# EmbersArc/EiCOS

Hardware: NVIDIA B200
Metric: SOCP solves/sec (higher is better)
Workload: dtype f64

## Files before the change

### eicos_b200/csrc/engine.cu

```cuda
#include "engine.hpp"
#include "backend.hpp"
#include "tile_program.hpp"

#include <algorithm>
#include <cstdint>
#ifdef EICOS_EMU
#include <thread>
#endif

namespace eicos
{

#ifndef EICOS_EMU
#define EI_DEFINE_KERNEL(name, fn, minblocks) EI_DEFINE_KERNEL_(name, fn, EI_MAX_THREADS, minblocks, 0)
#define EI_DEFINE_KERNEL1(name, fn) EI_DEFINE_KERNEL_(name, fn, 32, 8, 0)
#define EI_DEFINE_KERNEL_(name, fn, maxthreads, minblocks, JOBS)                                           \
    __global__ void __launch_bounds__(maxthreads, minblocks) name(const __grid_constant__ KArgs a) \
    {                                                                                          \
        extern __shared__ double smem[];                                                       \
        Team tm;                                                                               \
        tm.pl = threadIdx.x & 31;                                                              \
        tm.lane = tm.pl * VEC;                                                                 \
        tm.wk = threadIdx.x >> 5;                                                              \
        tm.nwk = blockDim.x >> 5;                                                              \
// ... 210 lines not shown
        P.Gp = upload(S.G.p, owned_, st);
        P.Gi = upload(S.G.i, owned_, st);
        P.Ap = upload(S.A.p, owned_, st);
        P.Ai = upload(S.A.i, owned_, st);
        P.Grp = upload(S.Gr.p, owned_, st);
        P.Grv = upload(S.Gr.v, owned_, st);
        P.Arp = upload(S.Ar.p, owned_, st);
        P.Arv = upload(S.Ar.v, owned_, st);
        P.cone_z = upload(S.cone_z, owned_, st);
    }
    P.cone_dim = upload(S.q, owned_, st);
    P.cone_k = upload(S.cone_k, owned_, st);
    P.cone_q = upload(S.cone_q, owned_, st);
    P.zk = upload(S.zk, owned_, st);
    P.xeq = dxeq_ = upload(S.xeq, owned_, st);
    P.Aeq = dAeq_ = upload(S.Aeq, owned_, st);
    P.GeqE = dGeq_ = upload(expanded_geq(S), owned_, st);
    const auto prog = [&](const MachineCode &h, DevMachine &d, int **keep = nullptr) {
        int *o = upload(h.ops, owned_, st);
        d.ops = o;
        d.nchunks = h.nchunks;
        d.nld_chunks = h.nld_chunks;
        d.ring_groups = h.ring_groups;
        d.ring_row0 = m_row_slot0(h.nr) + h.nr * h.slot_budget;
        if (keep)
            *keep = o;
    };
    const auto variant = [&](const ivec &list, std::initializer_list<int> va, std::initializer_list<int> vb = {}) {
        ivec out(list.size());
        int off[16] = {0};
        int k = 1;
        for (int o : va)
            off[k++] = o;
        k = 9;
        for (int o : vb)
            off[k++] = o;
        for (size_t q = 0; q < list.size(); q++)
        {
            const int w = list[q];
            out[q] = w == M_LD_NONE ? 0 : (w & M_LD_ROW_MASK) + off[(((unsigned)w >> M_LD_SEL_SHIFT) & 7) + ((w & M_LD_JOB_B) ? 8 : 0)];
        }
        return upload(out, owned_, st);
    };
    P.sw_budget = H_.fw[0].slot_budget;
    P.fa_budget = H_.fa[0].slot_budget;
    const int rhs[2] = {L_.rhs1, L_.rhs2}, sol[2] = {L_.sol1, L_.sol2}, xw[2] = {L_.xw, L_.xw2};
    const int dxr[2] = {L_.dxr, L_.dxr2}, er[2] = {L_.e, L_.e2};
    for (int v = 0; v < M_VARIANTS; v++)
    {
        prog(H_.fw[v], P.fw[v]);
        prog(H_.bw[v], P.bw[v]);
        prog(H_.bwp[v], P.bwp[v]);
        prog(H_.mv[v], P.mv[v], &dmv_ops_[v]);
        prog(H_.fa[v], P.fa[v], &dfa_ops_[v]);
        for (int set = 0; set < 2; set++)
        {
            P.fw_ld[v][set][0] = variant(H_.fw[v].ld, {rhs[set], 0, xw[set]});
            P.fw_ld[v][set][1] = variant(H_.fw[v].ld, {er[set], 0, xw[set]});
            P.bw_ld[v][set][0] = variant(H_.bwp[v].ld, {sol[set], 0, xw[set], rhs[set]});
            P.bw_ld[v][set][1] = variant(H_.bw[v].ld, {dxr[set], sol[set], xw[set], er[set]});
            P.mv_ld[v][set] = variant(H_.mv[v].ld, {rhs[set], sol[set], L_.lpv, er[set]});
        }
        P.fa_ld[v] = variant(H_.fa[v].ld, {});
    }
    for (int k = 0; k < M_MV_PARTS; k++)
    {
        prog(H_.rs[k], P.rs[k], &drs_ops_[k]);
        prog(H_.mvw[k], P.mvw[k], &dmvw_ops_[k]);
        P.rs_ld[k] = variant(H_.rs[k].ld, {L_.chb, L_.w, L_.s, L_.r, L_.sc});
        for (int set = 0; set < 2; set++)
            P.mvw_ld[set][k] = variant(H_.mvw[k].ld, {rhs[set], sol[set], L_.lpv, er[set]});
    }
    P.pair_budget = H_.pair_budget;
    prog(H_.fw2, P.fw2);
    prog(H_.bw2, P.bw2);
    prog(H_.bwp2, P.bwp2);
    prog(H_.mv2, P.mv2, &dmv2_ops_);
    P.fw2_ld[0] = variant(H_.fw2.ld, {rhs[0], 0, xw[0]}, {rhs[1], 0, xw[1]});
    P.fw2_ld[1] = variant(H_.fw2.ld, {er[0], 0, xw[0]}, {er[1], 0, xw[1]});
    P.bw2_ld[0] = variant(H_.bwp2.ld, {sol[0], 0, xw[0], rhs[0]}, {sol[1], 0, xw[1], rhs[1]});
    P.bw2_ld[1] = variant(H_.bw2.ld, {dxr[0], sol[0], xw[0], er[0]}, {dxr[1], sol[1], xw[1], er[1]});
    P.mv2_ld = variant(H_.mv2.ld, {rhs[0], sol[0], L_.lpv, er[0]}, {rhs[1], sol[1], L_.lpv, er[1]});
    P.mv_rows = H_.mv_rows;
    ivec vk;
    for (int k = 0; k < S.l; k++)
        vk.push_back(0);
    for (int d : S.q)
    {
        for (int k = 0; k < d + 1; k++)
            vk.push_back(0);
        for (int k = 1; k < d; k++)
            vk.push_back(1);
        vk.push_back(2);
        for (int k = 0; k < d; k++)
            vk.push_back(1);
    }
    P.Vkind = upload(vk, owned_, st);
    be::sync(st);
}

void Engine::upload_values(const Symbolic &S)
{
    be::stream_t st = S_(stream_);
    be::set_device(device_);
    refresh_stream_values(S, L_, H_, pim_);
    const dvec ge = expanded_geq(S);
    be::h2d(dxeq_, S.xeq.data(), S.xeq.size() * sizeof(double), st);
    be::h2d(dAeq_, S.Aeq.data(), S.Aeq.size() * sizeof(double), st);
    be::h2d(dGeq_, ge.data(), ge.size() * sizeof(double), st);
    for (int v = 0; v < M_VARIANTS; v++)
    {
        be::h2d(dmv_ops_[v], H_.mv[v].ops.data(), H_.mv[v].ops.size() * sizeof(int), st);
        be::h2d(dfa_ops_[v], H_.fa[v].ops.data(), H_.fa[v].ops.size() * sizeof(int), st);
    }
    be::h2d(dmv2_ops_, H_.mv2.ops.data(), H_.mv2.ops.size() * sizeof(int), st);
    for (int k = 0; k < M_MV_PARTS; k++)
    {
        be::h2d(drs_ops_[k], H_.rs[k].ops.data(), H_.rs[k].ops.size() * sizeof(int), st);
        be::h2d(dmvw_ops_[k], H_.mvw[k].ops.data(), H_.mvw[k].ops.size() * sizeof(int), st);
    }
    be::sync(st);
}

Engine::Engine(const Symbolic &S, int device, long long capacity_instances, int workers, bool instance_matrices)
    : device_(device), workers_(std::max(1, std::min(workers, EI_MAX_THREADS / 32 > 0 ? EI_MAX_THREADS / 32 : 1))),
      pim_(instance_matrices), nnzG_(S.G.nnz()), nnzA_(S.A.nnz())
{
    be::set_device(device_);
    if (const char *v = std::getenv("EICOS_RING_VARIANT"))
        force_variant_ = std::atoi(v);
    if (const char *v = std::getenv("EICOS_PAIR_SOLVES"))
        force_pair_ = std::atoi(v);
    if (const char *v = std::getenv("EICOS_WIDE"))
        force_wide_ = std::atoi(v);
    stream_ = (void *)(intptr_t)be::make_stream();
    build_layout(S, false);
    upload_pattern(S);
    cap_tiles_ = std::max<long long>(1, (capacity_instances + TILE - 1) / TILE);
    ws_bytes_ = (size_t)cap_tiles_ * L_.rows_total * TILE * sizeof(double);
    ws_ = (double *)be::alloc(ws_bytes_);
    const size_t ib = (size_t)cap_tiles_ * L_.irows_total * TILE * sizeof(int);
    iws_ = (int *)be::alloc(ib);
    be::zero(ws_, ws_bytes_, S_(stream_));
    be::zero(iws_, ib, S_(stream_));
    base_vec_ = (double *)be::alloc((size_t)(S.n + S.m + S.p) * sizeof(double));
    if (pim_)
        base_mat_ = (double *)be::alloc((size_t)(nnzG_ + nnzA_ + 1) * sizeof(double));
    active_count_ = (unsigned int *)be::alloc(sizeof(unsigned int));
    ir_rounds_ = (unsigned long long *)be::alloc(8 * sizeof(unsigned long long));
    host_pinned_ = (unsigned int *)be::pinned(12 * sizeof(unsigned long long));
    const size_t slots = (size_t)cap_tiles_ * TILE;
    moves_dev_ = (int *)be::alloc(2 * slots * sizeof(int));
    status_host_ = (int *)be::pinned(slots * sizeof(int));
    moves_host_ = (int *)be::pinned(2 * slots * sizeof(int));
    for (int v = 0; v < M_VARIANTS; v++)
    {
        const int sw_v = std::max(std::max(H_.fw[v].slot_budget, H_.bw[v].slot_budget), std::max(H_.bwp[v].slot_budget, H_.mv[v].slot_budget));
        smem_prog_[v] = machine_smem_doubles(sw_v, variant_groups(v)) * sizeof(double);
        smem_factor_[v] = machine_smem_doubles(P_.fa_budget, variant_groups(v)) * sizeof(double);
    }
    smem_pair_ = machine_smem_doubles(P_.pair_budget, M_PAIR_GROUPS, 2) * sizeof(double);
    part_doubles_ = machine_smem_doubles(P_.sw_budget, M_PART_GROUPS);
    smem_resid_ = part_doubles_ * sizeof(double);
    smem_wide_ = ((size_t)M_MV_PARTS * KRED * TILE +
                  std::max((size_t)M_MV_PARTS * part_doubles_, std::max(smem_prog_[0], smem_prog_[M_VARIANTS - 1]) / sizeof(double))) *
                 sizeof(double);
    smem_common_ = workers_ > 1 ? (size_t)workers_ * KRED * TILE * sizeof(double) : 0;
#ifndef EICOS_EMU
    {
        if (smem_pair_ > 48 * 1024)
            EI_CUDA(cudaFuncSetAttribute(eicos_solve_kkt_pair, cudaFuncAttributeMaxDynamicSharedMemorySize, (int)smem_pair_));
        if (smem_wide_ > 48 * 1024)
        {
            EI_CUDA(cudaFuncSetAttribute(eicos_solve_kkt_wide, cudaFuncAttributeMaxDynamicSharedMemorySize, (int)smem_wide_));
            EI_CUDA(cudaFuncSetAttribute(eicos_residuals_wide, cudaFuncAttributeMaxDynamicSharedMemorySize, (int)smem_wide_));
        }
        if (smem_resid_ > 48 * 1024)
            EI_CUDA(cudaFuncSetAttribute(eicos_residuals, cudaFuncAttributeMaxDynamicSharedMemorySize, (int)smem_resid_));
        const size_t top_f = std::max(smem_factor_[0], smem_factor_[M_VARIANTS - 1]), top_p = std::max(smem_prog_[0], smem_prog_[M_VARIANTS - 1]);
        if (top_f > 48 * 1024)
            EI_CUDA(cudaFuncSetAttribute(eicos_ldl_factor, cudaFuncAttributeMaxDynamicSharedMemorySize, (int)top_f));
        if (top_p > 48 * 1024)
        {
            EI_CUDA(cudaFuncSetAttribute(eicos_solve_kkt, cudaFuncAttributeMaxDynamicSharedMemorySize, (int)top_p));
            EI_CUDA(cudaFuncSetAttribute(eicos_residuals, cudaFuncAttributeMaxDynamicSharedMemorySize, (int)top_p));
        }
        int dev_sms = 148;
        EI_CUDA(cudaDeviceGetAttribute(&dev_sms, cudaDevAttrMultiProcessorCount, device_));
        sms_ = dev_sms;
    }
    if (smem_common_ > 48 * 1024)
    {
        const void *ks[] = {(const void *)eicos_load_inputs, (const void *)eicos_equilibrate, (const void *)eicos_init,
                            (const void *)eicos_init_point,
                            (const void *)eicos_iter_head, (const void *)eicos_iter_mid, (const void *)eicos_iter_tail,
                            (const void *)eicos_store_outputs};
        for (const void *k : ks)
            EI_CUDA(cudaFuncSetAttribute(k, cudaFuncAttributeMaxDynamicSharedMemorySize, (int)smem_common_));
    }
#endif
    be::sync(S_(stream_));
}

Engine::~Engine()
{
    be::set_device(device_);
#ifndef EICOS_EMU
    for (void *e : events_)
        cudaEventDestroy((cudaEvent_t)e);
#endif
    for (void *p : owned_)
        be::dfree(p);
    be::dfree(ws_);
    be::dfree(iws_);
    be::dfree(base_vec_);
    be::dfree(base_mat_);
    be::dfree(active_count_);
// ... 444 lines not shown
```

### eicos_b200/csrc/engine.hpp

```cpp
#pragma once

#include "layout.hpp"
#include "streams.hpp"
#include "symbolic.hpp"

#include <cstddef>
#include <vector>

namespace eicos
{

struct SolveStats
{
    int chunks = 0, compactions = 0;
    int ipm_iterations = 0;
    long long launches = 0;
    unsigned long long ir_rounds = 0;
    unsigned long long kkt_phase_cycles[5] = {0, 0, 0, 0, 0};
    double ms_total = 0, ms_factor = 0, ms_solve = 0, ms_other = 0;
    long long factor_launch_tiles = 0, solve_launch_tiles = 0;
    int factor_launches = 0, solve_launches = 0;
    double ms_resid = 0, ms_vector = 0;
    long long resid_launch_tiles = 0, vector_launch_tiles = 0;
    int resid_launches = 0, vector_launches = 0;
// ... 9 lines not shown
        factor_launch_tiles += o.factor_launch_tiles, solve_launch_tiles += o.solve_launch_tiles;
        factor_launches += o.factor_launches, solve_launches += o.solve_launches;
        ms_resid += o.ms_resid, ms_vector += o.ms_vector;
        resid_launch_tiles += o.resid_launch_tiles, vector_launch_tiles += o.vector_launch_tiles;
        resid_launches += o.resid_launches, vector_launches += o.vector_launches;
        lane_rounds += o.lane_rounds;
        return *this;
    }
};

struct ProgramStats
{
    int sw_slots = 0, fa_slots = 0, fa_fast = 0;
    long long sw_far = 0, sw_direct = 0, fa_home = 0;
    int fw_loads = 0, bw_loads = 0, fa_loads = 0, mv_loads = 0;
};

class Engine
{
  public:
    Engine(const Symbolic &S, int device, long long capacity_instances, int workers, bool instance_matrices = false);
    ~Engine();
    Engine(const Engine &) = delete;
    Engine &operator=(const Engine &) = delete;

    void set_matrices(const double *d_G, const double *d_A, const double *base_G, const double *base_A);
    bool instance_matrices() const { return pim_; }

    void upload_values(const Symbolic &S);

    void solve(int batch, const double *d_c, const double *d_h, const double *d_b,
               const double *base_c, const double *base_h, const double *base_b,
               double *d_x, double *d_y, double *d_z, double *d_s,
               int *d_exit, int *d_iter, double *d_info, int *d_iinfo,
               bool keep_sticky, bool pre_equilibrated, bool timing, SolveStats *stats);

    void debug_factor_init(int batch, const double *d_c, const double *d_h, const double *d_b,
                           const double *base_c, const double *base_h, const double *base_b,
                           double *h_Lx, double *h_D, double *h_sol1, double *h_sol2, int *h_nit);

    void debug_line_search(int batch, const double *h_lambda, const double *h_ds, const double *h_dz, const double *h_scalars,
                           double *h_alpha);

    ProgramStats program_stats() const;
    void *stream() const { return stream_; }
    int device() const { return device_; }
    int workers() const { return workers_; }
    void set_compaction(bool on) { compaction_ = on; }
    void set_iter_max(int k) { iter_max_ = k; }
    long long capacity() const { return cap_tiles_ * (long long)tile_width(); }
    size_t workspace_bytes() const { return ws_bytes_; }
    const Layout &layout() const { return L_; }
    static int tile_width();

  private:
    void build_layout(const Symbolic &S, bool acc_rows);
    void upload_pattern(const Symbolic &S);

    int device_ = 0, workers_ = 4;
    bool pim_ = false;
    const double *mat_dG_ = nullptr, *mat_dA_ = nullptr;
    double *base_mat_ = nullptr;
    int nnzG_ = 0, nnzA_ = 0;
    long long cap_tiles_ = 0;
    size_t ws_bytes_ = 0;
    void *stream_ = nullptr;
    Layout L_{};
    DevPattern P_{};
    double *ws_ = nullptr;
    int *iws_ = nullptr;
    double *base_vec_ = nullptr;
    unsigned int *active_count_ = nullptr;
    unsigned long long *ir_rounds_ = nullptr;
    unsigned int *host_pinned_ = nullptr;
    int *moves_dev_ = nullptr, *status_host_ = nullptr, *moves_host_ = nullptr;
    bool compaction_ = true;
    size_t smem_factor_[M_VARIANTS] = {0, 0}, smem_common_ = 0, smem_prog_[M_VARIANTS] = {0, 0};
    size_t smem_pair_ = 0;
    size_t smem_resid_ = 0, smem_wide_ = 0, part_doubles_ = 0;
    int force_wide_ = -1;
    int iter_max_ = Settings::iter_max;
    bool wide_launch(int ctas) const;
    int sms_ = 148, force_variant_ = -1, force_pair_ = -1;
    bool deep_ring(int ctas) const;
    bool pair_solves(int tiles) const;
    std::vector<void *> owned_;
    double *dxeq_ = nullptr, *dAeq_ = nullptr, *dGeq_ = nullptr;
    int *dmv_ops_[M_VARIANTS] = {nullptr, nullptr}, *drs_ops_[M_MV_PARTS] = {nullptr, nullptr, nullptr, nullptr}, *dmvw_ops_[M_MV_PARTS] = {nullptr, nullptr, nullptr, nullptr}, *dfa_ops_[M_VARIANTS] = {nullptr, nullptr}, *dmv2_ops_ = nullptr;
    HostStreams H_;
    std::vector<int> Lp_;
    std::vector<void *> events_;
};

}
```

### eicos_b200/csrc/layout.hpp

```cpp
#pragma once

#include <cstddef>

namespace eicos
{

enum : int
{
    ST_ACTIVE = -1000,
    EXIT_OPTIMAL = 0,
    EXIT_PINF = 1,
    EXIT_DINF = 2,
    EXIT_MAXIT = -1,
    EXIT_NUMERICS = -2,
    EXIT_OUTCONE = -3,
    EXIT_FATAL = -7,
    EXIT_INACC = 10,
    EXIT_NOT_CONVERGED = -87
};

enum ScalarRow : int
{
    S_KAP, S_TAU, S_CX, S_BY, S_HZ,
    S_PCOST, S_DCOST, S_PRES, S_DRES, S_PINFRES, S_DINFRES, S_GAP, S_RELGAP,
    S_SIGMA, S_MU, S_STEP, S_STEP_AFF, S_KAPOVERT,
    S_WORK_END,
    S_BEST = S_WORK_END,
    S_BEST_END = S_BEST + S_WORK_END,
    S_RT = S_BEST_END, S_NX, S_NY, S_NZ, S_NS, S_HRESX, S_HRESY, S_HRESZ,
    S_RESX0, S_RESY0, S_RESZ0, S_PRES_PREV,
    S_DTAU_DENOM, S_DTAUAFF, S_DKAPAFF,
    S_RHSMAX1, S_RHSMAX2,
    S_RED,
    S_COUNT = S_RED + 14
};

enum IntRow : int
{
    J_ITER, J_PINF, J_DINF, J_HAS_PINFRES, J_HAS_DINFRES, J_HAS_RELGAP, J_NIT1, J_NIT2, J_NIT3,
    J_WORK_END,
    J_BEST = J_WORK_END,
    J_BEST_END = J_BEST + J_WORK_END,
    J_STATUS = J_BEST_END,
    J_INST,
    J_STORED,
    J_COUNT
};

struct Layout
{
    int chb;
    int w;
    int s, lam;
    int wb, bs;
    int r;
    int lpv, lpw;
    int cpar, cq;
    int V;
    int Lx, D, Dinv;
    int rhs1, rhs2, sol1, sol2;
    int xw, dxr, e;
    int xw2, dxr2, e2;
    int dsw, wdz, dsaff, ds1;
    int Gx, Ax, eq;
    int sc;
    int acc;
    int rows_total;
    int irows_total;
};

struct DevMachine
{
    const int *ops;
    int nchunks;
    int nld_chunks;
    int ring_groups;
    int ring_row0;
};

enum ConeParam : int
{
    CP_ETA, CP_ETA2, CP_A, CP_D1, CP_U0, CP_U1, CP_V1, CP_W, CP_COUNT
};

struct DevPattern
{
    int n, p, m, l, nc, N, mt, qtot, nnzL, nnzV, maxcol;
    const int *cone_dim, *cone_k, *cone_q;
    const int *zk;
    const double *xeq, *Aeq, *GeqE;
    DevMachine fw[2], bw[2], bwp[2], mv[2];
    const int *fw_ld[2][2][2], *bw_ld[2][2][2], *mv_ld[2][2];
    DevMachine rs[4], mvw[4];
    const int *rs_ld[4], *mvw_ld[2][4];
    DevMachine fw2, bw2, bwp2, mv2;
    const int *fw2_ld[2], *bw2_ld[2], *mv2_ld;
    int mv_rows;
    int sw_budget, fa_budget, pair_budget;
    DevMachine fa[2];
    const int *fa_ld[2];
    int pim, nnzG, nnzA;
    const int *Gp, *Gi, *Ap, *Ai, *Grp, *Grv, *Arp, *Arv, *cone_z;
    const int *Vkind;
};

}
```

### eicos_b200/csrc/machine.cpp

```cpp
#include "machine.hpp"

#include <algorithm>
#include <climits>
#include <string>
#include <cstdint>
#include <cstring>
#include <cstdlib>
#include <queue>
#include <set>
#include <stdexcept>

namespace eicos
{
namespace
{
inline int field(int row) { return row << M_FIELD_SHIFT; }

void schedule(const MProgram &P, int window, std::vector<ivec> &bundles, ivec &bundle_of)
{
    const int n = (int)P.ops.size(), nv = (int)P.vals.size();
    ivec producer(nv, -1);
    for (int t = 0; t < n; t++)
        if (P.ops[t].dst >= 0)
        {
// ... 215 lines not shown
        }
    };

    struct Pending
    {
        int val;
        size_t k_at;
        size_t f_at;
    };
    for (int b = 0; b < (int)bundles.size(); b++)
    {
        {
            ivec &cur = bundles[b];
            int keep = 0, regular = NR - 1, reread = 0;
            for (; keep < (int)cur.size(); keep++)
            {
                int r1 = regular, r2 = reread;
                pops_of(P.ops[cur[keep]], r1, r2);
                if (keep > 0 && (r2 > 16 || r1 + r2 > RING_ROWS - 8))
                    break;
                regular = r1, reread = r2;
            }
            if (regular + reread > RING_ROWS - 8 || reread > 16)
                throw std::logic_error("machine: one operation pops more rows than the ring holds");
            if (keep < (int)cur.size())
            {
                ivec rest(cur.begin() + keep, cur.end());
                cur.resize(keep);
                for (int t : rest)
                    optime[t]++;
                bundles.insert(bundles.begin() + b + 1, rest);
            }
        }
        const ivec &cur = bundles[b];
        int pbmax = -1;
        for (int t : cur)
        {
            const MSrc *src[4] = {&P.ops[t].a, &P.ops[t].b, &P.ops[t].c, &P.ops[t].x3};
            for (const MSrc *s : src)
                if (s->kind == MS_VAL && slot_of[s->val] < 0)
                {
                    if (written_at[s->val] == -2)
                        throw std::logic_error("machine: value lost (neither in a slot nor at home)");
                    pbmax = std::max(pbmax, written_at[s->val]);
                }
        }
        if (pbmax >= 0)
            pad_to((first_pop[pbmax] / M_RING_GROUP + 2) * M_RING_GROUP);
        close_prev();
        first_pop.push_back(npop);
        const long long window_end = (first_pop[b] / M_RING_GROUP + RG) * M_RING_GROUP;

        const size_t rec0 = out.ops.size();
        out.ops.resize(rec0 + M_BUNDLE_WORDS, 0);
        struct Reread
        {
            size_t at;
            int val;
            bool vec, keep_b;
            size_t f_at, w5_at;
        };
        struct Load
        {
            size_t at;
            int word;
            bool vec;
        };
        std::vector<Load> loads;
        std::vector<Reread> rereads;
        std::vector<Pending> dsts;
        ivec last_used;
        for (int u = 0; u < M_U; u++)
        {
            const size_t r = rec0 + (size_t)u * M_REC_WORDS;
            int *w = out.ops.data() + r;
            if (u >= (int)cur.size())
            {
                w[0] = w[1] = w[2] = field(M_ROW_ZERO);
                w[3] = field(m_row_trash(NR));
                out.nnop++;
                continue;
            }
            const MOp &op = P.ops[cur[u]];
            out.nops++;
            int flags = op.flags;
            bool has_const = false;
            double cval = 0.0;
            const auto resolve = [&](const MSrc &s, int which) {
                const size_t at = r + (which == 3 ? 6 : which);
                const bool vec = which != 0;
                switch (s.kind)
                {
                case MS_ZERO:
                    out.ops[at] = field(M_ROW_ZERO);
                    break;
                case MS_NEGZERO:
                    out.ops[at] = field(m_row_negzero(NR));
                    break;
                case MS_LOAD:
                {
                    if (s.row < 0 || s.row > M_LD_ROW_MASK || s.sel < 0 || s.sel > 7)
                        throw std::logic_error("machine: load row out of range");
                    loads.push_back({at, (s.sel << M_LD_SEL_SHIFT) | s.row, vec && NR > 1});
                    break;
                }
                case MS_CONST:
                    if (which != 0 && which != 2)
                        throw std::logic_error("machine: constant in a B / x3 operand");
                    if (has_const)
                        throw std::logic_error("machine: two constants in one operation");
                    has_const = true;
                    cval = s.c;
                    flags |= which == 0 ? MF_ACONST : MF_CCONST;
                    out.ops[at] = field(M_ROW_ZERO);
                    break;
                case MS_VAL:
                {
                    const int v = s.val;
                    if (!vec && NR > 1)
                        throw std::logic_error("machine: a value as the A operand of a two-job program");
                    if (slot_of[v] >= 0)
                        out.ops[at] = field(slot_row(slot_of[v]));
                    else
                        rereads.push_back({at, v, vec, which == 1, r + 4, r + 5});
                    uptr[v]++;
                    if (uptr[v] == (int)uses[v].size())
                        last_used.push_back(v);
                    break;
                }
                }
            };
            if (op.x3.kind != MS_ZERO && (op.a.kind == MS_CONST || op.c.kind == MS_CONST))
                throw std::logic_error("machine: a functor operand and a constant in one operation");
            resolve(op.a, 0);
            resolve(op.b, 1);
            resolve(op.c, 2);
            if (op.x3.kind != MS_ZERO)
            {
                resolve(op.x3, 3);
                flags |= MF_X3;
            }
            if (has_const)
            {
                int32_t cw[2];
                std::memcpy(cw, &cval, sizeof(cval));
                w = out.ops.data() + r;
                w[6] = cw[0];
                w[7] = cw[1];
            }
            w = out.ops.data() + r;
            w[3] = field(m_row_trash(NR));
            w[4] = flags;
            w[5] = (flags & MF_OUT) ? op.out_row : 0;
            if (op.dst >= 0)
                dsts.push_back({op.dst, r + 3, r + 4});
        }
        {
            size_t next_single = 0;
            const auto place_single = [&]() {
                while (next_single < loads.size() && loads[next_single].vec)
                    next_single++;
                if (next_single == loads.size())
                    return false;
                out.ops[loads[next_single].at] = field(push_single(loads[next_single].word));
                next_single++;
                return true;
// ... 340 lines not shown
```

### eicos_b200/csrc/machine.hpp

```cpp
#pragma once

#include "symbolic.hpp"

#include <stdexcept>
#include <vector>

namespace eicos
{

#ifndef EICOS_M_U
#define EICOS_M_U 4
#endif
constexpr int M_U = EICOS_M_U;
constexpr int M_REC_WORDS = 8;
constexpr int M_BUNDLE_WORDS = M_U * M_REC_WORDS;
constexpr int M_CHUNK_BUNDLES = 8;
constexpr int M_CHUNK_WORDS = M_CHUNK_BUNDLES * M_BUNDLE_WORDS;
constexpr int M_CHUNKS = 2;
constexpr int M_RING_GROUP = 8;
constexpr int M_MAX_RING_GROUPS = 16;
constexpr int M_ROW_ZERO = 0;
constexpr int m_row_negzero(int nr) { return nr; }
constexpr int m_row_trash(int nr) { return 2 * nr; }
constexpr int m_row_slot0(int nr) { return 3 * nr; }
// ... 27 lines not shown
};

enum MSrcKind : int
{
    MS_ZERO,
    MS_NEGZERO,
    MS_VAL,
    MS_LOAD,
    MS_CONST
};
struct MSrc
{
    int kind = MS_ZERO;
    int val = -1;
    int sel = 0, row = 0;
    double c = 0.0;
    static MSrc zero() { return MSrc(); }
    static MSrc negzero()
    {
        MSrc s;
        s.kind = MS_NEGZERO;
        return s;
    }
    static MSrc value(int v)
    {
        MSrc s;
        s.kind = MS_VAL;
        s.val = v;
        return s;
    }
    static MSrc load(int sel, int row)
    {
        MSrc s;
        s.kind = MS_LOAD;
        s.sel = sel;
        s.row = row;
        return s;
    }
    static MSrc constant(double c)
    {
        MSrc s;
        s.kind = MS_CONST;
        s.c = c;
        return s;
    }
};
struct MOp
{
    MSrc a, b, c, x3;
    int dst = -1;
    int flags = 0;
    int out_row = 0;
};
struct MVal
{
    int home_sel = -1;
    int home_row = 0;
};
struct MProgram
{
    std::vector<MOp> ops;
    std::vector<MVal> vals;
    bool keep_loads = false;
    int nr = 1;
    int new_value(int home_sel = -1, int home_row = 0)
    {
        MVal v;
        v.home_sel = home_sel;
        v.home_row = home_row;
        vals.push_back(v);
        return (int)vals.size() - 1;
    }
};

struct MachineOutOfSlots : std::runtime_error
{
    using std::runtime_error::runtime_error;
};

struct MachineCode
{
    ivec ops;
    ivec ld;
    int nbundles = 0, nchunks = 0, nld = 0, nld_chunks = 0;
    int nr = 1;
    int ring_groups = 4;
    int slot_budget = 0;
    int window = 0;
    int slot_rows = 0;
    long long nops = 0, nnop = 0;
    long long far = 0, pads = 0, spills = 0;
};

void machine_compile(const MProgram &P, int max_slots, MachineCode &out, int tune_slots = 0, int ring_groups = 4, int window = 0);

}
```

### eicos_b200/csrc/streams.cpp

```cpp
#include "streams.hpp"

#include <algorithm>
#include <cstdint>
#include <cstdio>
#include <cstdlib>
#include <cstring>
#include <stdexcept>

namespace eicos
{
namespace
{

void build_forward(const Symbolic &S, const Layout &L, MProgram &P)
{
    ivec xval(S.N, -1);
    for (int i = 0; i < S.N; i++)
    {
        const int t0 = S.Lr.p[i], cnt = S.Lr.p[i + 1] - t0;
        if (cnt == 0)
        {
            xval[i] = P.new_value(1, S.pinv[i]);
            continue;
        }
// ... 191 lines not shown
        const auto link = [&]() {
            if (ci == chains.size())
                return false;
            P.ops.push_back(chains[ci][cq]);
            if (++cq == chains[ci].size())
                ci++, cq = 0;
            return true;
        };
        for (const MOp &op : shorts)
        {
            P.ops.push_back(op);
            if (gap && ++since >= gap)
            {
                since = 0;
                link();
            }
        }
        while (link())
        {
        }
    }
    mv_rows = (int)R.order.size();
}

void build_resid(const Symbolic &S, const Layout &L, MProgram &P, bool pim, int part, int parts)
{
    MatvecRows R;
    matvec_rows(S, L, R);
    size_t first, last;
    matvec_part(R, part, parts, first, last);
    const int zb = S.n + S.p;
    P.keep_loads = true;
    ivec xv(S.N);
    for (int c = 0; c < S.N; c++)
        xv[c] = P.new_value(2, c);
    const int tau_home = P.new_value(5, S_TAU);
    const int tau = P.new_value(-1, 0);
    {
        MOp op;
        op.c = MSrc::value(tau_home);
        op.dst = tau;
        P.ops.push_back(op);
    }
    for (size_t at = first; at < last; at++)
    {
        const int r = R.order[at];
        const int kind = mv_kind(S, r);
        const bool zrow = kind >= MV_Z;
        const int pre = kind == MV_X ? RS_PRE_X : (kind == MV_Y ? RS_PRE_Y : RS_PRE_Z);
        const int fin = kind == MV_X ? RS_FIN_X : (kind == MV_Y ? RS_FIN_Y : RS_FIN_Z);
        const size_t cnt = R.ent[r].size();
        int prev = -1;
        if (zrow)
        {
            MOp op;
            op.c = MSrc::load(3, r - zb);
            op.x3 = MSrc::value(xv[r]);
            op.flags |= MF_FIN | ((cnt == 0 ? RS_FIRST_PRE_Z : RS_FIRST_Z) << MF_KIND_SHIFT);
            op.dst = prev = P.new_value(4, r);
            P.ops.push_back(op);
        }
        for (size_t q = 0; q < cnt; q++)
        {
            MOp op;
            op.c = prev >= 0 ? MSrc::value(prev) : MSrc::zero();
            op.a = pim ? MSrc::load(0, R.crow[r][q]) : MSrc::constant(R.ent[r][q].second);
            op.b = MSrc::value(xv[R.ent[r][q].first]);
            if (kind != MV_X)
                op.flags |= MF_POS;
            if (q + 1 == cnt)
                op.flags |= MF_FIN | (pre << MF_KIND_SHIFT);
            op.dst = prev = P.new_value(4, r);
            P.ops.push_back(op);
        }
        MOp op;
        op.c = prev >= 0 ? MSrc::value(prev) : MSrc::zero();
        op.a = MSrc::value(tau);
        op.b = MSrc::load(1, r);
        op.x3 = MSrc::value(xv[r]);
        op.flags |= MF_OUT | MF_FIN | (fin << MF_KIND_SHIFT);
        op.out_row = r;
        op.dst = P.new_value(4, r);
        P.ops.push_back(op);
    }
}

ivec ag_rows(const Symbolic &S, const Layout &L)
{
    ivec row(S.Ki.size(), -1);
    for (size_t k = 0; k < S.AGslot.size(); k++)
        row[S.AGslot[k]] = S.AGsrc[k] >= 0 ? L.Ax + S.AGsrc[k] : L.Gx + (-S.AGsrc[k] - 1);
    return row;
}

void build_factor(const Symbolic &S, const Layout &L, MProgram &P, bool pim)
{
    struct Init
    {
        int kind = 0;
        int vrow = -1;
        double c = 0.0;
    };
    const ivec agrow = pim ? ag_rows(S, L) : ivec(S.Ki.size(), -1);
    std::vector<Init> di(S.N), ei(S.nnzL);
    for (int j = 0; j < S.N; j++)
        for (int e = S.KLp[j]; e < S.KLp[j + 1]; e++)
        {
            const int slot = S.KLslot[e], vi = S.Kvidx[slot], pos = S.KLpos[e];
            Init &t = pos < 0 ? di[j] : ei[S.Lp[j] + pos];
            if (vi >= 0 || agrow[slot] >= 0)
            {
                t.kind = 2;
                t.vrow = vi >= 0 ? L.V + vi : agrow[slot];
            }
            else
            {
                t.kind = 1;
                t.c = S.Kshared[slot];
            }
        }
    P.keep_loads = true;
    ivec dcur(S.N, -1), ecur(S.nnzL, -1);
    const auto start = [&](const Init &t) {
        return t.kind == 2 ? MSrc::load(0, t.vrow) : (t.kind == 1 ? MSrc::constant(t.c) : MSrc::zero());
    };
    std::vector<MSrc> av, lv;
    for (int k = 0; k < S.N; k++)
    {
        const int u0 = S.Lp[k], cnt = S.Lp[k + 1] - u0;
        int rd;
        {
            MOp op;
            op.c = dcur[k] >= 0 ? MSrc::value(dcur[k]) : start(di[k]);
            op.flags |= MF_RECIP | MF_OUT | MF_FIN | (FIN_PIVOT << MF_KIND_SHIFT);
            op.out_row = L.Dinv + k;
            op.dst = rd = P.new_value(0, L.Dinv + k);
            P.ops.push_back(op);
        }
        if (cnt == 0)
            continue;
        av.assign(cnt, MSrc());
        lv.assign(cnt, MSrc());
        for (int e = 0; e < cnt; e++)
        {
            const Init &t = ei[u0 + e];
            if (ecur[u0 + e] >= 0)
                av[e] = MSrc::value(ecur[u0 + e]);
            else if (t.kind == 2)
                av[e] = MSrc::value(P.new_value(0, t.vrow));
            else
                av[e] = MSrc::constant(t.kind == 1 ? t.c : 0.0);
            MOp op;
            op.c = MSrc::negzero();
            op.flags |= MF_POS | MF_OUT;
            op.out_row = L.Lx + u0 + e;
            if (av[e].kind == MS_CONST)
            {
                op.a = av[e];
                op.b = MSrc::value(rd);
            }
            else
            {
                op.a = MSrc::value(rd);
                op.b = av[e];
            }
            op.dst = P.new_value(0, L.Lx + u0 + e);
// ... 12 lines not shown
                {
                    const int i2 = S.Li[u0 + e2];
                    const int *b = S.Li.data() + S.Lp[i2], *e = S.Li.data() + S.Lp[i2 + 1];
                    const int *f = std::lower_bound(b, e, i1);
                    if (f == e || *f != i1)
                        throw std::logic_error("factor program: update outside the pattern of L");
                    const int ut = (int)(f - S.Li.data());
                    cur = &ecur[ut];
                    init = &ei[ut];
                    home = L.acc >= 0 ? L.acc + ut : -1;
                }
                else
                {
                    cur = &dcur[i1];
                    init = &di[i1];
                    home = L.D + i1;
                }
                MOp op;
                op.c = *cur >= 0 ? MSrc::value(*cur) : start(*init);
                if (op.c.kind == MS_CONST && av[e1].kind == MS_CONST)
                {
                    MOp mv;
                    mv.c = op.c;
                    mv.dst = P.new_value(home >= 0 ? 0 : -1, std::max(home, 0));
                    P.ops.push_back(mv);
                    op.c = MSrc::value(mv.dst);
                }
                if (av[e1].kind == MS_CONST)
                {
                    op.a = av[e1];
                    op.b = lv[e2];
                }
                else
                {
                    op.a = lv[e2];
                    op.b = av[e1];
                }
                op.dst = *cur = P.new_value(home >= 0 ? 0 : -1, std::max(home, 0));
                P.ops.push_back(op);
            }
        }
    }
}
}

void build_streams(const Symbolic &S, const Layout &L, int W, int max_sw_slots, int max_fa_slots, HostStreams &H, bool pim)
{
    constexpr int MACHINE_TUNE_SLOTS = 16, MACHINE_TUNE_FA_SLOTS = 24;
    H = HostStreams();
    H.workers = W;
    H.sw_budget = max_sw_slots;
    H.fa_budget = max_fa_slots;
    for (int k = 0; k < S.N; k++)
        for (int u = S.Lp[k]; u + 1 < S.Lp[k + 1]; u++)
            if (S.Li[u] >= S.Li[u + 1])
                throw std::logic_error("columns of L must have ascending rows");
    if (S.fma_count > MAX_FACTOR_UPDATES)
        throw std::runtime_error("pattern fills too much for the row-program factorisation (" + std::to_string(S.fma_count) +
                                 " Schur updates per factorisation; limit " + std::to_string(MAX_FACTOR_UPDATES) + ")");
    {
        const int slots = std::max(2, max_sw_slots);
        MProgram pf, pb, pbp, pm;
        build_forward(S, L, pf);
        build_backward(S, L, pb, true);
        build_backward(S, L, pbp, false);
        build_matvec(S, L, pm, H.mv_rows, pim);
        const auto compile = [&](const char *name, const MProgram &p, MachineCode (&c)[M_VARIANTS], int budget, int tune, int deep = 0) {
            const std::string key = std::string("EICOS_SCHED_WINDOW_") + name;
            const char *v = std::getenv(key.c_str());
            machine_compile(p, budget, c[0], tune, variant_groups(0), v ? std::max(M_U, std::atoi(v)) : 0);
            for (int k = 1; k < M_VARIANTS; k++)
                machine_compile(p, deep > 0 ? deep : budget, c[k], tune, variant_groups(k), c[0].window);
            if (std::getenv("EICOS_DBG_PROGRAMS"))
                for (int k = 0; k < M_VARIANTS; k++)
                    std::fprintf(stderr, "machine %s[%d]: ops %lld nop %lld bundles %d loads %d far %lld pads %lld spills %lld slots %d window %d\n",
                                 name, k, c[k].nops, c[k].nnop, c[k].nbundles, c[k].nld, c[k].far, c[k].pads, c[k].spills, c[k].slot_rows,
                                 c[k].window);
        };
        const int deep_slots = std::getenv("EICOS_MAX_SW_SLOTS") ? slots : 2 * slots;
        compile("fw", pf, H.fw, slots, MACHINE_TUNE_SLOTS, deep_slots);
        compile("bw", pb, H.bw, slots, MACHINE_TUNE_SLOTS, deep_slots);
        compile("bwp", pbp, H.bwp, slots, MACHINE_TUNE_SLOTS, deep_slots);
        compile("mv", pm, H.mv, slots, MACHINE_TUNE_SLOTS, deep_slots);
        for (int k = 0; k < M_MV_PARTS; k++)
        {
            MProgram pr, pw;
            int rows_unused = 0;
            build_resid(S, L, pr, pim, k, M_MV_PARTS);
            build_matvec(S, L, pw, rows_unused, pim, k, M_MV_PARTS);
            machine_compile(pr, slots, H.rs[k], MACHINE_TUNE_SLOTS, M_PART_GROUPS, 0);
            machine_compile(pw, slots, H.mvw[k], MACHINE_TUNE_SLOTS, M_PART_GROUPS, 0);
            if (std::getenv("EICOS_DBG_PROGRAMS"))
                for (auto nq : {std::make_pair("rs", &H.rs[k]), std::make_pair("mvw", &H.mvw[k])})
                    std::fprintf(stderr, "machine %s part %d: ops %lld nop %lld bundles %d loads %d far %lld pads %lld spills %lld slots %d window %d\n",
                                 nq.first, k, nq.second->nops, nq.second->nnop, nq.second->nbundles, nq.second->nld, nq.second->far,
                                 nq.second->pads, nq.second->spills, nq.second->slot_rows, nq.second->window);
        }
        {
            const int pslots = std::max(2, std::min(14, max_sw_slots * 14 / 16));
            H.pair_budget = pslots;
            const auto pair = [&](const char *name, MProgram &p, MachineCode &c, int window) {
                p.nr = 2;
                machine_compile(p, pslots, c, 0, M_PAIR_GROUPS, window);
                if (std::getenv("EICOS_DBG_PROGRAMS"))
                    std::fprintf(stderr, "machine %s: ops %lld nop %lld bundles %d loads %d far %lld pads %lld spills %lld slots %d window %d\n", name,
                                 c.nops, c.nnop, c.nbundles, c.nld, c.far, c.pads, c.spills, c.slot_rows, c.window);
            };
            pair("fw2", pf, H.fw2, H.fw[0].window);
            pair("bw2", pb, H.bw2, H.bw[0].window);
            pair("bwp2", pbp, H.bwp2, H.bwp[0].window);
            pair("mv2", pm, H.mv2, H.mv[0].window);
        }
        MProgram pa;
        build_factor(S, L, pa, pim);
        compile("fa", pa, H.fa, std::max(2, max_fa_slots), MACHINE_TUNE_FA_SLOTS);
        for (int k = 0; k < M_VARIANTS; k++)
            for (const MachineCode *q : {&H.fw[k], &H.bw[k], &H.bwp[k], &H.mv[k]})
                H.sw_slots = std::max(H.sw_slots, q->slot_rows);
        for (int k = 0; k < M_MV_PARTS; k++)
            H.sw_slots = std::max(H.sw_slots, std::max(H.rs[k].slot_rows, H.mvw[k].slot_rows));
        H.sw_far = H.fw[0].far + H.bwp[0].far;
        H.fa_slots = std::max(H.fa[0].slot_rows, H.fa[1].slot_rows);
        H.fa_home = H.fa[0].spills + H.fa[0].far;
    }
}

void refresh_stream_values(const Symbolic &S, const Layout &L, HostStreams &H, bool pim)
{
    HostStreams fresh;
    build_streams(S, L, H.workers, std::max(H.sw_budget, 2), std::max(H.fa_budget, 2), fresh, pim);
    std::vector<std::pair<MachineCode *, MachineCode *>> pq = {{&H.mv2, &fresh.mv2}};
    for (int k = 0; k < M_VARIANTS; k++)
        for (auto q : {std::make_pair(&H.mv[k], &fresh.mv[k]), std::make_pair(&H.fa[k], &fresh.fa[k])})
            pq.push_back(q);
    for (int k = 0; k < M_MV_PARTS; k++)
        for (auto q : {std::make_pair(&H.rs[k], &fresh.rs[k]), std::make_pair(&H.mvw[k], &fresh.mvw[k])})
            pq.push_back(q);
    for (auto &q : pq)
    {
        if (q.second->ops.size() != q.first->ops.size())
            throw std::logic_error("machine program changed shape on a value refresh");
        q.first->ops.swap(q.second->ops);
    }
}

}
```

### eicos_b200/csrc/streams.hpp

```cpp
#pragma once

#include "layout.hpp"
#include "machine.hpp"
#include "symbolic.hpp"

#include <algorithm>
#include <cstdlib>
#include <string>
#include <vector>

namespace eicos
{

constexpr int M_VARIANTS = 2;
constexpr int M_VARIANT_GROUPS[M_VARIANTS] = {3, 5};
inline int variant_groups(int v)
{
    if (v == 0)
        if (const char *e = std::getenv("EICOS_SHALLOW_GROUPS"))
            return std::max(2, std::min(M_MAX_RING_GROUPS, std::atoi(e)));
    return M_VARIANT_GROUPS[v];
}
constexpr int M_PAIR_GROUPS = 3;
constexpr int M_MV_PARTS = 4;
constexpr int M_PART_GROUPS = 4;

constexpr long long MAX_FACTOR_UPDATES = 20LL * 1000 * 1000;

enum MvKind : int
{
    MV_X = 0,
    MV_Y = 1,
    MV_Z = 2,
    MV_ZC = 3
};
enum : int
{
    FIN_ACC = 1,
    FIN_ABSMAX = 2,
    RS_PRE_X = 3, RS_PRE_Y, RS_PRE_Z, RS_FIN_X, RS_FIN_Y, RS_FIN_Z, RS_FIRST_Z, RS_FIRST_PRE_Z,
    FIN_PIVOT = 11
};

struct HostStreams
{
    int workers = 1;
    int sw_budget = 0, fa_budget = 0;
    MachineCode fw[M_VARIANTS], bw[M_VARIANTS], bwp[M_VARIANTS], mv[M_VARIANTS];
    MachineCode rs[M_MV_PARTS], mvw[M_MV_PARTS];
    int mv_rows = 0;
    MachineCode fa[M_VARIANTS];
    MachineCode fw2, bw2, bwp2, mv2;
    int pair_budget = 0;
    int sw_slots = 0, fa_slots = 0;
    long long sw_far = 0, fa_home = 0;
};

void build_streams(const Symbolic &S, const Layout &L, int workers, int max_sw_slots, int max_fa_slots, HostStreams &H,
                   bool pim = false);

void refresh_stream_values(const Symbolic &S, const Layout &L, HostStreams &H, bool pim = false);

}
```

### eicos_b200/csrc/tile_program.hpp

```cpp
#pragma once

#include "layout.hpp"
#include "streams.hpp"
#include "symbolic.hpp"

#include <cfloat>
#include <cmath>

#ifdef EICOS_EMU
#include <barrier>
#define EI_DEV inline
#define EI_LDG(p) (*(p))
#define EI_CLOCK() 0ll
#else
#include <cuda_runtime.h>
#define EI_DEV __device__ __forceinline__
#define EI_LDG(p) __ldg(p)
#define EI_CLOCK() clock64()
#endif

#ifndef EICOS_VEC
#define EICOS_VEC 2
#endif

// ... 977 lines not shown
                issue_group();
            if (last)
                break;
        }
#if EICOS_TMA_RING
        while (gwaited < lgroup)
            wait_next_group();
#else
        asm volatile("cp.async.wait_all;" ::: "memory");
#endif
        for (int c = cons + 1; c < fetched; c++)
            mbar_wait(bars + 8u * ((unsigned)c % M_CHUNKS), ((unsigned)c / M_CHUNKS) & 1u);
        for (int c = (lgroup + M_LD_CHUNK_GROUPS - 1) / M_LD_CHUNK_GROUPS; c < ld_fetched; c++)
            mbar_wait(bars + 8u * (M_CHUNKS + (unsigned)c % M_LD_CHUNKS), ((unsigned)c / M_LD_CHUNKS) & 1u);
        __syncwarp();
        if (pl == 0)
            for (int b = 0; b < M_CHUNKS + M_LD_CHUNKS + (EICOS_TMA_RING ? M_MAX_RING_GROUPS : 0); b++)
                mbar_inval(bars + 8u * b);
        __syncwarp();
    }
#endif
};

struct NoFin
{
    template <int NR>
    EI_DEV void operator()(int, int, const vd (&)[NR], const vd (&)[NR], const vd (&)[NR]) {}
};

struct PivotFin
{
    vb zero_pivot;
    EI_DEV void operator()(int, int, const vd (&res)[1], const vd (&)[1], const vd (&)[1])
    {
        VFOR zero_pivot.v[c_] = zero_pivot.v[c_] || fabs(res[0].v[c_]) > DBL_MAX;
    }
};
EI_DEV void tile_factor(const Team &tm, const KArgs &a, int tile)
{
    const TileMem t = tile_mem(tm, a, tile);
    const vb act = lane_active(tm, t);
    if (!tm.any(act))
        return;
    if (tm.wk != 0)
        return;
    Machine mm;
    mm.init(tm, tm.pbuf);
    PivotFin fin;
    fin.zero_pivot = vbset(false);
    MRun r;
    r.prog = a.P.fa[a.variant];
    r.ld = a.P.fa_ld[a.variant];
    r.Tb = t.Tb;
    r.out = r.out2 = r.outB = r.out2B = t.T;
    r.a_one = false;
    mm.run<MC_CONST | MC_POS | MC_BKEEP | MC_RECIP | MC_FIN, 1>(tm, r, fin);
    VFOR if (fin.zero_pivot.v[c_] && act.v[c_]) ROWC(t.I, J_STATUS, c_) = EXIT_FATAL;
}

template <int NR>
struct AccFin
{
    vb cont[NR];
    double *x[NR];
    EI_DEV void operator()(int, int row, const vd (&res)[NR], const vd (&)[NR], const vd (&xa)[NR])
    {
#pragma unroll
        for (int j = 0; j < NR; j++)
            vstore(x[j] + (size_t)row * TILE, xa[j] + vsel(cont[j], res[j], vset(0.0)));
    }
};
template <int NR>
struct AbsMaxFin
{
    vd nerr[NR];
    EI_DEV void operator()(int, int, const vd (&res)[NR], const vd (&)[NR], const vd (&)[NR])
    {
#pragma unroll
        for (int j = 0; j < NR; j++)
            nerr[j] = vmax(nerr[j], vabs(res[j]));
    }
};

template <int NR>
EI_DEV void kkt_residual(const Team &tm, const KArgs &a, Machine &mm, const TileMem &t, const DevMachine &prog, const int *mvld,
                         const int (&x)[NR], const int (&erow)[NR], bool initialize, vd (&nerr)[NR], int set = 0)
{
    const DevPattern &P = a.P;
    const Layout &L = a.L;
    double *T = t.T;
    const double delta = Settings::deltastat;
    const int zb = P.n + P.p;
#pragma unroll
    for (int j = 0; j < NR; j++)
        nerr[j] = vset(0.0);
    const bool wide = NR == 1 && tm.nwk >= M_MV_PARTS;
    if ((wide ? tm.wk < M_MV_PARTS : tm.wk == 0) && P.mv_rows > 0)
    {
        AbsMaxFin<NR> fin;
#pragma unroll
        for (int j = 0; j < NR; j++)
            fin.nerr[j] = vset(0.0);
        Machine mw;
        if (wide)
            mw.init(tm, tm.pbuf + (size_t)tm.wk * a.part_doubles);
        Machine &mrun = wide ? mw : mm;
        MRun r;
        r.prog = wide ? P.mvw[tm.wk] : prog;
        r.ld = wide ? P.mvw_ld[set][tm.wk] : mvld;
        r.Tb = t.Tb;
        r.out = r.out2 = T + (size_t)erow[0] * TILE;
        r.outB = r.out2B = T + (size_t)erow[NR - 1] * TILE;
        r.a_one = false;
        mrun.template run<MC_CONST | MC_BKEEP | MC_FIN, NR>(tm, r, fin);
#pragma unroll
        for (int j = 0; j < NR; j++)
            nerr[j] = fin.nerr[j];
    }
    if (P.nc > 0)
    {
        tm.sync();
        for (int c = tm.wk; c < P.nc; c += tm.nwk)
        {
            const int d = EI_LDG(P.cone_dim + c), ks = EI_LDG(P.cone_k + c), qo = EI_LDG(P.cone_q + c);
            const int kb = zb + ks;
            const int cp = L.cpar + c * CP_COUNT;
            const vd eta2 = ROWD(T, cp + CP_ETA2), d1 = ROWD(T, cp + CP_D1), u0 = ROWD(T, cp + CP_U0);
            const vd u1 = ROWD(T, cp + CP_U1), v1 = ROWD(T, cp + CP_V1);
            for (int j = 0; j < NR; j++)
            {
                const int xj = x[j], ej = erow[j];
                const vd x1 = ROWD(T, xj + kb), x3 = ROWD(T, xj + kb + d), x4 = ROWD(T, xj + kb + d + 1);
                vd qtx2 = vset(0.0);
                for (int k = 1; k < d; k++)
                    qtx2 += vd(ROWD(T, L.cq + qo + k - 1)) * vd(ROWD(T, xj + kb + k));
                const vd vu = v1 * x3 + u1 * x4;
                for (int k = 0; k < d; k++)
                {
                    const vd xk = ROWD(T, xj + kb + k);
                    vd v = ROWD(T, ej + kb + k);
                    if (k < d - 1)
                        v += delta * xk;
                    else
                        v -= delta * xk;
                    if (initialize)
                        v += xk;
                    else if (k == 0)
                        v += eta2 * (d1 * x1 + u0 * x4);
                    else
                        v += eta2 * (xk + vu * vd(ROWD(T, L.cq + qo + k - 1)));
                    ROWD(T, ej + kb + k) = v;
                    nerr[j] = vmax(nerr[j], vabs(v));
                }
                const vd e3 = initialize ? x3 : eta2 * (v1 * qtx2 + x3);
                const vd e4 = initialize ? x4 : eta2 * (u0 * x1 + u1 * qtx2 - x4);
                ROWD(T, ej + kb + d) = e3;
                ROWD(T, ej + kb + d + 1) = e4;
                nerr[j] = vmax(nerr[j], vmax(vabs(e3), vabs(e4)));
            }
        }
    }
    team_max<NR>(tm, nerr);
}

template <int NR>
EI_DEV void tile_solve_kkt(const Team &tm, const KArgs &a, int tile)
{
    const TileMem t = tile_mem(tm, a, tile);
    const vb act = lane_active(tm, t);
    if (!tm.any(act))
        return;
    const DevPattern &P = a.P;
    const Layout &L = a.L;
    double *T = t.T;
    const bool init = a.initialize != 0;
    int sol[NR], xw[NR], dxr[NR], erow[NR], nitrow[NR];
    vd threshold[NR];
#pragma unroll
    for (int j = 0; j < NR; j++)
    {
        const KArgs::KktJob jb = a.job[NR == 1 ? tm.job : j];
        const int set = jb.set;
        sol[j] = jb.sol;
        nitrow[j] = jb.nitrow;
        xw[j] = set ? L.xw2 : L.xw;
        dxr[j] = set ? L.dxr2 : L.dxr;
        erow[j] = set ? L.e2 : L.e;
        threshold[j] = (1. + vd(ROWD(T, L.sc + (set ? S_RHSMAX2 : S_RHSMAX1)))) * Settings::linsysacc;
    }
    const int set0 = a.job[NR == 1 ? tm.job : 0].set, v = a.variant;
    const DevMachine &pfw = NR == 1 ? P.fw[v] : P.fw2, &pbw = NR == 1 ? P.bw[v] : P.bw2;
    const DevMachine &pbwp = NR == 1 ? P.bwp[v] : P.bwp2, &pmv = NR == 1 ? P.mv[v] : P.mv2;
    const int *fw_ld[2], *bw_ld[2], *mv_ld;
    if (NR == 1)
    {
        fw_ld[0] = P.fw_ld[v][set0][0], fw_ld[1] = P.fw_ld[v][set0][1];
        bw_ld[0] = P.bw_ld[v][set0][0], bw_ld[1] = P.bw_ld[v][set0][1];
// ... 1342 lines not shown
```

Baseline: 45790.

## Evaluate wide refinement residual mat-vec from a direct record list

```diff
diff --git a/eicos_b200/csrc/engine.cu b/eicos_b200/csrc/engine.cu
--- a/eicos_b200/csrc/engine.cu
+++ b/eicos_b200/csrc/engine.cu
@@ -316,6 +316,12 @@
     P.bw2_ld[1] = variant(H_.bw2.ld, {dxr[0], sol[0], xw[0], er[0]}, {dxr[1], sol[1], xw[1], er[1]});
     P.mv2_ld = variant(H_.mv2.ld, {rhs[0], sol[0], L_.lpv, er[0]}, {rhs[1], sol[1], L_.lpv, er[1]});
     P.mv_rows = H_.mv_rows;
+    P.mvl[0] = P.mvl[1] = nullptr;
+    if (matvec_direct_ && !H_.mvl.rec.empty())
+        for (int set = 0; set < 2; set++)
+            P.mvl[set] = dmvl_[set] = upload(direct_list(H_.mvl, {rhs[set], sol[set], L_.lpv, er[set]}), owned_, st);
+    for (int k = 0; k <= M_MV_PARTS; k++)
+        P.mvl_part[k] = H_.mvl.part[k];
     ivec vk;
     for (int k = 0; k < S.l; k++)
         vk.push_back(0);
@@ -331,6 +337,25 @@
     }
     P.Vkind = upload(vk, owned_, st);
     be::sync(st);
+}
+
+ivec Engine::direct_list(const MvList &M, std::initializer_list<int> rows) const
+{
+    int off[8] = {0};
+    int k = 1;
+    for (int o : rows)
+        off[k++] = o;
+    const auto row = [&](int w) { return w == M_LD_NONE ? -1 : (w & M_LD_ROW_MASK) + off[((unsigned)w >> M_LD_SEL_SHIFT) & 7]; };
+    ivec out;
+    out.reserve(4 * M.rec.size());
+    for (const MvRec &r : M.rec)
+    {
+        int w[2] = {row(r.out), r.fin};
+        if ((r.type & (MVD_LAST - 1)) != MVD_HEAD)
+            std::memcpy(w, &r.coef, sizeof(double));
+        out.insert(out.end(), {row(r.row), r.type, w[0], w[1]});
+    }
+    return out;
 }
 
 void Engine::upload_values(const Symbolic &S)
@@ -353,6 +378,14 @@
         be::h2d(drs_ops_[k], H_.rs[k].ops.data(), H_.rs[k].ops.size() * sizeof(int), st);
         be::h2d(dmvw_ops_[k], H_.mvw[k].ops.data(), H_.mvw[k].ops.size() * sizeof(int), st);
     }
+    const int rhs[2] = {L_.rhs1, L_.rhs2}, sol[2] = {L_.sol1, L_.sol2}, er[2] = {L_.e, L_.e2};
+    ivec lists[2];
+    for (int set = 0; set < 2; set++)
+        if (dmvl_[set])
+        {
+            lists[set] = direct_list(H_.mvl, {rhs[set], sol[set], L_.lpv, er[set]});
+            be::h2d(dmvl_[set], lists[set].data(), lists[set].size() * sizeof(int), st);
+        }
     be::sync(st);
 }
 
@@ -367,6 +400,8 @@
         force_pair_ = std::atoi(v);
     if (const char *v = std::getenv("EICOS_WIDE"))
         force_wide_ = std::atoi(v);
+    if (const char *v = std::getenv("EICOS_MATVEC"))
+        matvec_direct_ = std::atoi(v) != 0;
     stream_ = (void *)(intptr_t)be::make_stream();
     build_layout(S, false);
     upload_pattern(S);
diff --git a/eicos_b200/csrc/engine.hpp b/eicos_b200/csrc/engine.hpp
--- a/eicos_b200/csrc/engine.hpp
+++ b/eicos_b200/csrc/engine.hpp
@@ -115,11 +115,14 @@
     int iter_max_ = Settings::iter_max;
     bool wide_launch(int ctas) const;
     int sms_ = 148, force_variant_ = -1, force_pair_ = -1;
+    bool matvec_direct_ = true;
+    ivec direct_list(const MvList &M, std::initializer_list<int> rows) const;
     bool deep_ring(int ctas) const;
     bool pair_solves(int tiles) const;
     std::vector<void *> owned_;
     double *dxeq_ = nullptr, *dAeq_ = nullptr, *dGeq_ = nullptr;
     int *dmv_ops_[M_VARIANTS] = {nullptr, nullptr}, *drs_ops_[M_MV_PARTS] = {nullptr, nullptr, nullptr, nullptr}, *dmvw_ops_[M_MV_PARTS] = {nullptr, nullptr, nullptr, nullptr}, *dfa_ops_[M_VARIANTS] = {nullptr, nullptr}, *dmv2_ops_ = nullptr;
+    int *dmvl_[2] = {nullptr, nullptr};
     HostStreams H_;
     std::vector<int> Lp_;
     std::vector<void *> events_;
diff --git a/eicos_b200/csrc/layout.hpp b/eicos_b200/csrc/layout.hpp
--- a/eicos_b200/csrc/layout.hpp
+++ b/eicos_b200/csrc/layout.hpp
@@ -96,6 +96,8 @@
     DevMachine fw2, bw2, bwp2, mv2;
     const int *fw2_ld[2], *bw2_ld[2], *mv2_ld;
     int mv_rows;
+    const int *mvl[2];
+    int mvl_part[5];
     int sw_budget, fa_budget, pair_budget;
     DevMachine fa[2];
     const int *fa_ld[2];
diff --git a/eicos_b200/csrc/machine.cpp b/eicos_b200/csrc/machine.cpp
--- a/eicos_b200/csrc/machine.cpp
+++ b/eicos_b200/csrc/machine.cpp
@@ -321,6 +321,7 @@
                 continue;
             }
             const MOp &op = P.ops[cur[u]];
+            out.order.push_back(cur[u]);
             out.nops++;
             int flags = op.flags;
             bool has_const = false;
diff --git a/eicos_b200/csrc/machine.hpp b/eicos_b200/csrc/machine.hpp
--- a/eicos_b200/csrc/machine.hpp
+++ b/eicos_b200/csrc/machine.hpp
@@ -133,6 +133,7 @@
 {
     ivec ops;
     ivec ld;
+    ivec order;
     int nbundles = 0, nchunks = 0, nld = 0, nld_chunks = 0;
     int nr = 1;
     int ring_groups = 4;
diff --git a/eicos_b200/csrc/streams.cpp b/eicos_b200/csrc/streams.cpp
--- a/eicos_b200/csrc/streams.cpp
+++ b/eicos_b200/csrc/streams.cpp
@@ -297,6 +297,51 @@
         op.out_row = r;
         op.dst = P.new_value(4, r);
         P.ops.push_back(op);
+    }
+}
+
+int ld_word(int sel, int row) { return (sel << M_LD_SEL_SHIFT) | row; }
+ivec finish_order(const MProgram &P, const MachineCode &c)
+{
+    ivec rows;
+    for (int t : c.order)
+        if (P.ops[t].flags & MF_OUT)
+            rows.push_back(P.ops[t].out_row);
+    return rows;
+}
+void list_matvec(const Symbolic &S, const MatvecRows &R, const ivec &rows, MvList &M)
+{
+    const int zb = S.n + S.p;
+    for (int r : rows)
+    {
+        const int kind = mv_kind(S, r);
+        MvRec h;
+        h.type = MVD_HEAD;
+        h.row = ld_word(1, r);
+        h.out = ld_word(4, r);
+        h.fin = kind != MV_ZC;
+        M.rec.push_back(h);
+        const auto ent = [&](int row, double coef) {
+            MvRec e;
+            e.type = MVD_ENT;
+            e.row = row;
+            e.coef = coef;
+            M.rec.push_back(e);
+        };
+        for (const auto &en : R.ent[r])
+            ent(ld_word(2, en.first), -en.second);
+        if (kind != MV_ZC)
+            ent(ld_word(2, r), kind == MV_X ? -Settings::deltastat : Settings::deltastat);
+        if (kind == MV_Z)
+        {
+            MvRec e;
+            e.type = MVD_LPV;
+            e.row = ld_word(3, r - zb);
+            M.rec.push_back(e);
+        }
+        if (M.rec.back().type == MVD_HEAD)
+            ent(M_LD_NONE, -0.0);
+        M.rec.back().type |= MVD_LAST;
     }
 }
 
@@ -475,6 +520,8 @@
         compile("bw", pb, H.bw, slots, MACHINE_TUNE_SLOTS, deep_slots);
         compile("bwp", pbp, H.bwp, slots, MACHINE_TUNE_SLOTS, deep_slots);
         compile("mv", pm, H.mv, slots, MACHINE_TUNE_SLOTS, deep_slots);
+        MatvecRows R;
+        matvec_rows(S, L, R);
         for (int k = 0; k < M_MV_PARTS; k++)
         {
             MProgram pr, pw;
@@ -483,12 +530,19 @@
             build_matvec(S, L, pw, rows_unused, pim, k, M_MV_PARTS);
             machine_compile(pr, slots, H.rs[k], MACHINE_TUNE_SLOTS, M_PART_GROUPS, 0);
             machine_compile(pw, slots, H.mvw[k], MACHINE_TUNE_SLOTS, M_PART_GROUPS, 0);
+            if (!pim)
+            {
+                list_matvec(S, R, finish_order(pw, H.mvw[k]), H.mvl);
+                H.mvl.part[k + 1] = (int)H.mvl.rec.size();
+            }
             if (std::getenv("EICOS_DBG_PROGRAMS"))
                 for (auto nq : {std::make_pair("rs", &H.rs[k]), std::make_pair("mvw", &H.mvw[k])})
                     std::fprintf(stderr, "machine %s part %d: ops %lld nop %lld bundles %d loads %d far %lld pads %lld spills %lld slots %d window %d\n",
                                  nq.first, k, nq.second->nops, nq.second->nnop, nq.second->nbundles, nq.second->nld, nq.second->far,
                                  nq.second->pads, nq.second->spills, nq.second->slot_rows, nq.second->window);
         }
+        if (std::getenv("EICOS_DBG_PROGRAMS"))
+            std::fprintf(stderr, "direct refinement residual: %zu records\n", H.mvl.rec.size());
         {
             const int pslots = std::max(2, std::min(14, max_sw_slots * 14 / 16));
             H.pair_budget = pslots;
@@ -535,6 +589,9 @@
             throw std::logic_error("machine program changed shape on a value refresh");
         q.first->ops.swap(q.second->ops);
     }
-}
-
-}
+    if (fresh.mvl.rec.size() != H.mvl.rec.size())
+        throw std::logic_error("mat-vec row list changed shape on a value refresh");
+    H.mvl.rec.swap(fresh.mvl.rec);
+}
+
+}
diff --git a/eicos_b200/csrc/streams.hpp b/eicos_b200/csrc/streams.hpp
--- a/eicos_b200/csrc/streams.hpp
+++ b/eicos_b200/csrc/streams.hpp
@@ -42,6 +42,27 @@
     FIN_PIVOT = 11
 };
 
+enum : int
+{
+    MVD_HEAD = 1,
+    MVD_ENT,
+    MVD_LPV,
+    MVD_LAST = 8
+};
+struct MvRec
+{
+    int type = 0;
+    int row = M_LD_NONE;
+    int out = 0;
+    int fin = 0;
+    double coef = 0.0;
+};
+struct MvList
+{
+    std::vector<MvRec> rec;
+    int part[M_MV_PARTS + 1] = {0, 0, 0, 0, 0};
+};
+
 struct HostStreams
 {
     int workers = 1;
@@ -49,6 +70,7 @@
     MachineCode fw[M_VARIANTS], bw[M_VARIANTS], bwp[M_VARIANTS], mv[M_VARIANTS];
     MachineCode rs[M_MV_PARTS], mvw[M_MV_PARTS];
     int mv_rows = 0;
+    MvList mvl;
     MachineCode fa[M_VARIANTS];
     MachineCode fw2, bw2, bwp2, mv2;
     int pair_budget = 0;
diff --git a/eicos_b200/csrc/tile_program.hpp b/eicos_b200/csrc/tile_program.hpp
--- a/eicos_b200/csrc/tile_program.hpp
+++ b/eicos_b200/csrc/tile_program.hpp
@@ -1083,6 +1083,79 @@
     }
 };
 
+constexpr int MVD_D = 8;
+template <class Fin>
+EI_DEV void matvec_direct(const int *list, int k0, int k1, double *T, Fin &fin)
+{
+    const auto rec = [&](int k) {
+        i4 r;
+        r.x = -1, r.y = 0, r.z = 0, r.w = 0;
+        if (k < k1)
+            r = ldg4(list + 4 * (size_t)k);
+        return r;
+    };
+    const auto opnd = [&](const i4 &r) { return r.x >= 0 ? vload(T + (size_t)r.x * TILE) : vset(0.0); };
+    i4 rc[MVD_D], rn[MVD_D];
+    vd pc[MVD_D], pn[MVD_D];
+#pragma unroll
+    for (int u = 0; u < MVD_D; u++)
+        rc[u] = rec(k0 + u);
+#pragma unroll
+    for (int u = 0; u < MVD_D; u++)
+        pc[u] = opnd(rc[u]);
+#pragma unroll
+    for (int u = 0; u < MVD_D; u++)
+        rn[u] = rec(k0 + MVD_D + u);
+    vd v = vset(0.0), x = vset(0.0);
+    int out = 0, fin_row = 0;
+    for (int k = k0; k < k1; k += MVD_D)
+    {
+#pragma unroll
+        for (int u = 0; u < MVD_D; u++)
+            pn[u] = opnd(rn[u]);
+        i4 rr[MVD_D];
+#pragma unroll
+        for (int u = 0; u < MVD_D; u++)
+            rr[u] = rec(k + 2 * MVD_D + u);
+#pragma unroll
+        for (int u = 0; u < MVD_D; u++)
+        {
+            const i4 r = rc[u];
+            const vd p = pc[u];
+            const int ty = r.y & (MVD_LAST - 1);
+            if (ty == MVD_HEAD)
+            {
+                v = p;
+                out = r.z;
+                fin_row = r.w;
+            }
+            else if (ty == MVD_ENT)
+            {
+                x = p;
+                v = vfma(vset(words_double(r.z, r.w)), x, v);
+            }
+            else if (ty == MVD_LPV)
+                v = vfma(-p, x, v);
+            if (r.y & MVD_LAST)
+            {
+                vstore(T + (size_t)out * TILE, v);
+                if (fin_row)
+                {
+                    const vd rv[1] = {v};
+                    fin(FIN_ABSMAX, out, rv, rv, rv);
+                }
+            }
+        }
+#pragma unroll
+        for (int u = 0; u < MVD_D; u++)
+        {
+            rc[u] = rn[u];
+            pc[u] = pn[u];
+            rn[u] = rr[u];
+        }
+    }
+}
+
 template <int NR>
 EI_DEV void kkt_residual(const Team &tm, const KArgs &a, Machine &mm, const TileMem &t, const DevMachine &prog, const int *mvld,
                          const int (&x)[NR], const int (&erow)[NR], bool initialize, vd (&nerr)[NR], int set = 0)
@@ -1102,18 +1175,28 @@
 #pragma unroll
         for (int j = 0; j < NR; j++)
             fin.nerr[j] = vset(0.0);
-        Machine mw;
-        if (wide)
-            mw.init(tm, tm.pbuf + (size_t)tm.wk * a.part_doubles);
-        Machine &mrun = wide ? mw : mm;
-        MRun r;
-        r.prog = wide ? P.mvw[tm.wk] : prog;
-        r.ld = wide ? P.mvw_ld[set][tm.wk] : mvld;
-        r.Tb = t.Tb;
-        r.out = r.out2 = T + (size_t)erow[0] * TILE;
-        r.outB = r.out2B = T + (size_t)erow[NR - 1] * TILE;
-        r.a_one = false;
-        mrun.template run<MC_CONST | MC_BKEEP | MC_FIN, NR>(tm, r, fin);
+        bool direct = false;
+        if constexpr (NR == 1)
+            if (wide && P.mvl[set])
+            {
+                direct = true;
+                matvec_direct(P.mvl[set], P.mvl_part[tm.wk], P.mvl_part[tm.wk + 1], T, fin);
+            }
+        if (!direct)
+        {
+            Machine mw;
+            if (wide)
+                mw.init(tm, tm.pbuf + (size_t)tm.wk * a.part_doubles);
+            Machine &mrun = wide ? mw : mm;
+            MRun r;
+            r.prog = wide ? P.mvw[tm.wk] : prog;
+            r.ld = wide ? P.mvw_ld[set][tm.wk] : mvld;
+            r.Tb = t.Tb;
+            r.out = r.out2 = T + (size_t)erow[0] * TILE;
+            r.outB = r.out2B = T + (size_t)erow[NR - 1] * TILE;
+            r.a_one = false;
+            mrun.template run<MC_CONST | MC_BKEEP | MC_FIN, NR>(tm, r, fin);
+        }
 #pragma unroll
         for (int j = 0; j < NR; j++)
             nerr[j] = fin.nerr[j];
```

New measurement: 45810, median of 6. No clear change (+0.0%).
